# singhhp1069/charon

Hardware: AMD Instinct MI355X
Metric: verified+aggregated 3-of-4 threshold BLS sigs/sec at 1/2/4/8 MI355X (higher is better)
Workload: dtype u32 (Fp 14x28-bit limbs); 1 GPU; config2: 3-of-4, 10000 DVs x 1 attestation per GPU; parallelism=shard1, inflight_launches=3, batches_per_launch=16, rlc_group=16, rlc_chunk=8, gident=0, subgroup_batch=0, level0=passed, hw_queues=4

## Files before the change

charon_amd/csrc/bls_pair.h:

```cpp
#pragma once
#include "bls_lines.h"

namespace tbg {

TBG_HD Fp pair_mul_lane(uint32_t par, const Fp& a, const Fp& ap, const Fp& b, const Fp& bp) {
  const Fp nbp = fp_neg_l(bp);
  return fp_mul2(a, fp_select(par != 0, bp, b), ap, fp_select(par != 0, b, nbp));
}
TBG_HD Fp pair_sqr_lane(uint32_t par, const Fp& a, const Fp& ap) {
  const Fp x = fp_add_l(fp_select(par != 0, ap, a), ap);
  const Fp y = fp_select(par != 0, a, fp_sub_l(a, ap));
  return fp_mul(x, y);
}
TBG_HD Fp pair_conj_lane(uint32_t par, const Fp& a) { return fp_select(par != 0, fp_neg(a), a); }
TBG_HD Fp pair_mul_xi_lane(uint32_t par, const Fp& a, const Fp& ap) {
  return fp_select(par != 0, fp_add(a, ap), fp_sub(a, ap));
}
TBG_HD Fp pair_inv_lane(uint32_t par, const Fp& a, const Fp& ap) {
  const Fp t = fp_inv(fp_mul2(a, a, ap, ap));
  return fp_mul(pair_conj_lane(par, a), t);
}
TBG_HD Fp pair_const(uint32_t par, const Fp2Const& c) { return par ? fp_from_const(c.c1) : fp_from_const(c.c0); }

struct Fp2p { Fp c0, c1; };
// ... 258 lines not shown
TBG_DEV Fp2x px_conj(const Fp2x& a) { return {pair_conj_lane(pair_par(), a.v)}; }
TBG_DEV Fp2x px_mul_xi(const Fp2x& a) { return {pair_mul_xi_lane(pair_par(), a.v, pair_xch(a.v))}; }
TBG_DEV Fp2x px_mul_const(const Fp2x& a, const Fp2Const& c) {
  const uint32_t par = pair_par();
  return {pair_mul_lane(par, a.v, pair_xch(a.v), pair_const(par, c), pair_const(par ^ 1u, c))};
}
TBG_DEV Fp2x rlc_mul_c(const Fp2x& a, const Fp& c) { return {fp_mul(a.v, c)}; }
TBG_DEV Fp2x f_mulfp(const Fp2x& a, const Fp& c) { return {fp_mul(a.v, c)}; }
TBG_DEV Fp2x f_conj(const Fp2x& a) { return px_conj(a); }
TBG_DEV Fp2x f_mulc(const Fp2x& a, const Fp2Const& c) { return px_mul_const(a, c); }
template <> TBG_HD Fp2x f_zero<Fp2x>() { return {fp_zero()}; }
template <> TBG_HD Fp2x f_one<Fp2x>() {
#if defined(__HIP_DEVICE_COMPILE__)
  return {(threadIdx.x & 1u) ? fp_zero() : fp_one()};
#else
  return {fp_one()};
#endif
}

TBG_DEV Fp2x px_load(const Fp2& a) { return {(&a.c0)[pair_par()]}; }
TBG_DEV void px_store(Fp2& dst, const Fp2x& a) { (&dst.c0)[pair_par()] = a.v; }
TBG_DEV Aff<Fp2x> px_load(const G2A& a) { return {px_load(a.x), px_load(a.y)}; }
TBG_DEV Jac<Fp2x> px_load(const G2J& p) { return {px_load(p.X), px_load(p.Y), px_load(p.Z)}; }
TBG_DEV void px_store(G2A& dst, const Aff<Fp2x>& a) { px_store(dst.x, a.x); px_store(dst.y, a.y); }
TBG_DEV void px_store(G2J& dst, const Jac<Fp2x>& p) { px_store(dst.X, p.X); px_store(dst.Y, p.Y); px_store(dst.Z, p.Z); }
TBG_DEV void px_line_store(uint32_t* dst, const LineG<Fp2x>& l) {
  const uint32_t par = pair_par();
  const Fp* f[3] = {&l.l0.v, &l.l1.v, &l.l4.v};
#pragma unroll
  for (int k = 0; k < 3; ++k)
#pragma unroll
    for (int i = 0; i < NL; ++i) dst[(2 * k + par) * NL + i] = f[k]->l[i];
}

template <bool EVAL = true>
TBG_DEV void px_g2_lines(const Aff<Fp2x>& Q, const Fp& nxP, const Fp& yP, uint32_t* out) {
  Jac<Fp2x> T = jac_from_aff(Q);
  const uint32_t par = pair_par();
  uint32_t* dst = out;
  auto sink = [&](int k, const Fp2x& v) {
#pragma unroll
    for (int i = 0; i < NL; ++i) dst[(2 * k + par) * NL + i] = v.v.l[i];
  };
  for (int i = 62; i >= 0; --i) {
    miller_dbl_s<Fp2x, EVAL>(T, nxP, yP, sink);
    dst += LINE_WORDS;
    if ((X_ABS >> i) & 1) {
      miller_add_s<Fp2x, EVAL>(T, Q, nxP, yP, sink);
      dst += LINE_WORDS;
    }
  }
}

TBG_DEV Fp2 px_gather(const Fp2x& a) {
  const Fp o = pair_xch(a.v);
  return pair_par() ? Fp2{o, a.v} : Fp2{a.v, o};
}

}
#endif
```

charon_amd/csrc/bls_row.h:

```cpp
#pragma once
#include "bls_quad.h"

namespace tbg {

#if defined(__HIP_DEVICE_COMPILE__)
constexpr int ROW_N = 1;
#else
constexpr int ROW_N = 16;
#endif

template <class T>
struct RowV {
  T v[ROW_N];
};
using R32 = RowV<int32_t>;
using R64 = RowV<int64_t>;

template <class T, class F>
TBG_HD RowV<T> rmap(F&& f) {
  RowV<T> r;
#pragma unroll
  for (int k = 0; k < ROW_N; ++k) r.v[k] = f(k);
  return r;
}
// ... 451 lines not shown
}
TBG_HD void rl_add5(int r, RowLineSlots& S) {
  if (r >= 4) return;
  R32 a0, a1, b0, b1;
  if (r < 2) { a0 = rl_ld(S, RL_Y); a1 = rl_ld(S, RL_Y + 1); b0 = rl_p(S, 3, 0); b1 = rl_p(S, 3, 1); }
  else {
    a0 = r_norm(rl_p(S, 3, 2) - rl_aX3(S, 0));
    a1 = r_norm(rl_p(S, 3, 3) - rl_aX3(S, 1));
    b0 = rl_R(S, 0);
    b1 = rl_R(S, 1);
  }
  rl_job(S, 4, r, a0, a1, b0, b1);
}
TBG_HD void rl_add6(int r, RowLineSlots& S, int buf) {
  if (r >= 12) return;
  const int c = r & 1, j = r >> 1;
  if (j == 0) row_st(S.s[RL_X + c], row_reduce(rl_aX3(S, c)));
  else if (j == 1) row_st(S.s[RL_Y + c], row_reduce(rl_p(S, 4, 2 + c) - rl_p(S, 4, c)));
  else if (j == 2) row_st(S.s[RL_Z + c], rl_p(S, 2, 2 + c));
  else if (j == 3) row_st(S.l[buf][c], row_reduce(rl_p(S, 3, 6 + c) - rl_p(S, 3, 4 + c)));
  else if (j == 4) row_st(S.l[buf][2 + c], rl_p(S, 2, 6 + c));
  else row_st(S.l[buf][4 + c], rl_p(S, 3, 8 + c));
}

TBG_HD void rl_line_out(const RowLineSlots& S, int buf, int k, uint32_t* dst) {
  const Fp v = fp_from_signed(S.l[buf][k]);
  for (int i = 0; i < NL; ++i) dst[k * NL + i] = v.l[i];
}

template <class Exec, class Out>
TBG_HD void row_g2_lines(Exec& ex, Out& out6, RowLineSlots& S) {
  int idx = 0, buf = 0;
#pragma unroll 1
  for (int i = 62; i >= 0; --i) {
    ex([&](int r) { rl_dbl1(r, S); });
    ex([&](int r) { rl_dbl2(r, S); });
    ex([&](int r) { rl_dbl3(r, S); });
    ex([&](int r) { rl_dbl4(r, S, buf); });
    out6(buf, idx++);
    buf ^= 1;
    if ((X_ABS >> i) & 1) {
      ex([&](int r) { rl_add1(r, S); });
      ex([&](int r) { rl_add2(r, S); });
      ex([&](int r) { rl_add3(r, S); });
      ex([&](int r) { rl_add4(r, S); });
      ex([&](int r) { rl_add5(r, S); });
      ex([&](int r) { rl_add6(r, S, buf); });
      out6(buf, idx++);
      buf ^= 1;
    }
  }
}

}
```

charon_amd/csrc/k_msm.hip:

```cpp
#define TBG_ADD_DBL_INLINE 1
#ifndef TBG_SCHED_FENCE
#define TBG_SCHED_FENCE 1
#endif
#include "tbls_launch.h"
#include "bls_msm.h"
#include "bls_pair.h"
#include "bls_batchinv.h"

namespace tbg {

__global__ void __launch_bounds__(BINV_BLOCK) k_pubkey_tables(const G1A* pk, const G1A* xpk, const int32_t* status,
                                                              uint32_t n, G1A* tab) {
  const uint32_t i = blockIdx.x * blockDim.x + threadIdx.x;
  const bool in = i < n;
  const bool ok = in && status[i] == DEC_OK;
  G1A p0{fp_zero(), fp_zero()}, x0 = p0;
  if (ok) {
    p0 = pk[i];
    x0 = xpk[i];
  }
#if TBG_PK_W2
#pragma unroll 1
  for (int k = 0; k < (int)PK_TAB; ++k) {
    const G1J e = ok ? rlc_key_table_w2_entry(p0, x0, k) : jac_inf<Fp>();
    G1A a{fp_zero(), fp_zero()};
    const bool got = block_jac_to_aff<BINV_WAVES>(e, ok, a);
    if (in) tab[(size_t)PK_TAB * i + k] = got ? a : G1A{fp_zero(), fp_zero()};
  }
#else
  const Fp t = block_batch_inv<BINV_WAVES>(fp_reduce(fp_sub(x0.x, p0.x)), ok);
  if (!in) return;
  G1A ap{fp_zero(), fp_zero()}, am = ap;
  if (ok) rlc_pair_from_inv(p0, x0, t, ap, am);
  tab[2ull * i] = ap;
  tab[2ull * i + 1] = am;
#endif
}

__global__ void TBG_LAUNCH k_rlc_g1_l0(DevBatch B, const G1A* tab, const int32_t* pk_status, uint32_t n_pk) {
  const uint32_t i = blockIdx.x * blockDim.x + threadIdx.x;
  if (i >= B.n_partials || B.partial_status[i] != TBG_PS_NOT_VERIFIED) return;
  const uint32_t pid = B.pubkey_ids[i];
  const bool fused = l0_fused(B);
  if (pid >= n_pk || pk_status[pid] != DEC_OK) {
    B.partial_status[i] = TBG_PS_ERR_PUBKEY;
    if (fused) B.counters[CNT_L0_BAD] = 1;
    return;
  }
  if (fused) {
    const uint4 v = *(const uint4*)(B.l0f_u + 4ull * i);
    const uint32_t uf[4] = {v.x, v.y, v.z, v.w};
    B.part_p[i] = rlc_mul_key_l0f(tab + (size_t)PK_TAB * pid, fp_from_const(G1_BETA), uf);
    return;
  }
  const uint64_t r = rlc_scalar(B.rlc_seed, i);
  uint32_t u[4];
  rlc_digits(r, u);
  B.msm_r[i] = r;
  B.part_p[i] = rlc_mul_key(tab + (size_t)PK_TAB * pid, u);
#pragma unroll
// ... 82 lines not shown
    const int top = 31 - __builtin_clz(m);
#pragma unroll 1
    for (int bit = top - 1; bit >= 0; --bit) {
      acc = jac_dbl_in(acc);
      if ((m >> bit) & 1u) {
        __asm__ __volatile__("" ::: "memory");
        const Jac<Fp2x> b = px_load(B.msm_bkt[j]);
        acc = FAST ? jac_add_x(acc, b, exc) : jac_add(acc, b);
      }
    }
  }
  return acc;
}
#ifndef TBG_MSM_BUCKET_X
#define TBG_MSM_BUCKET_X 1
#endif
__device__ __noinline__ Jac<Fp2x> msm_bucket_complete(const DevBatch& B, uint32_t j) {
  bool unused = false;
  return msm_bucket_scaled<false>(B, j, unused);
}

__global__ void TBG_LAUNCH_N(TBG_PAIR_WAVES) k_msm_bucket(DevBatch B) {
  TBG_URGENT();
  const uint32_t j = (blockIdx.x * blockDim.x + threadIdx.x) >> 1;
  if (j >= MSM_BUCKETS) return;
  if (B.counters[CNT_L0_BAD]) return;
#if TBG_MSM_BUCKET_X
  bool exc = false;
  Jac<Fp2x> acc = msm_bucket_scaled<true>(B, j, exc);
  if (!pair_all(!exc)) acc = msm_bucket_complete(B, j);
#else
  Jac<Fp2x> acc = px_load(B.msm_part[MSM_SPLIT * j]);
#pragma unroll 1
  for (uint32_t sl = 1; sl < MSM_SPLIT; ++sl) acc = jac_add_in<Fp2x, true>(acc, px_load(B.msm_part[MSM_SPLIT * j + sl]));
  const uint32_t m = 2 * j + 1;
  if (m > 1 && !jac_is_inf(acc)) {
    const Jac<Fp2x> b = acc;
    const int top = 31 - __builtin_clz(m);
#pragma unroll 1
    for (int bit = top - 1; bit >= 0; --bit) {
      acc = jac_dbl_in(acc);
      if ((m >> bit) & 1u) acc = jac_add_in<Fp2x, true>(acc, b);
    }
  }
#endif
  px_store(B.msm_bkt[j], acc);
}

constexpr uint32_t MSM_TREE_PAIRS = 128;
constexpr uint32_t MSM_TREE_PER = 4;
constexpr uint32_t MSM_TREE_WG = MSM_BUCKETS / (MSM_TREE_PAIRS * MSM_TREE_PER);
static_assert(MSM_TREE_WG <= 2 * 64 && MSM_TREE_WG <= MSM_SUM_ENTRIES, "second tree kernel: one workgroup");

template <uint32_t PAIRS>
__device__ __forceinline__ Jac<Fp2x> pair_tree_sum(Jac<Fp2x> acc, Jac<Fp2x>* lds) {
  const uint32_t t = threadIdx.x, pr = t >> 1;
#pragma unroll 1
  for (uint32_t s = 1; s < PAIRS; s <<= 1) {
    lds[t] = acc;
    __syncthreads();
    if ((pr & (2 * s - 1)) == 0 && pr + s < PAIRS) acc = jac_add_in<Fp2x, true>(acc, lds[t + 2 * s]);
    __syncthreads();
  }
  return acc;
}

__global__ void __launch_bounds__(2 * MSM_TREE_PAIRS) k_msm_tree(DevBatch B) {
  TBG_URGENT();
  __shared__ Jac<Fp2x> lds[2 * MSM_TREE_PAIRS];
  if (B.counters[CNT_L0_BAD]) return;
  const uint32_t pr = threadIdx.x >> 1;
  const uint32_t a0 = (blockIdx.x * MSM_TREE_PAIRS + pr) * MSM_TREE_PER;
  Jac<Fp2x> acc = px_load(B.msm_bkt[a0]);
#pragma unroll 1
  for (uint32_t a = a0 + 1; a < a0 + MSM_TREE_PER; ++a) acc = jac_add_in<Fp2x, true>(acc, px_load(B.msm_bkt[a]));
  acc = pair_tree_sum<MSM_TREE_PAIRS>(acc, lds);
  if (pr == 0) px_store(B.msm_sum[blockIdx.x], acc);
}

__global__ void __launch_bounds__(MSM_TREE_WG) k_msm_tree_final(DevBatch B) {
  TBG_URGENT();
  constexpr uint32_t PAIRS = MSM_TREE_WG / 2;
  __shared__ Jac<Fp2x> lds[2 * PAIRS];
  if (B.counters[CNT_L0_BAD]) return;
  const uint32_t pr = threadIdx.x >> 1;
  Jac<Fp2x> acc = jac_add_in<Fp2x, true>(px_load(B.msm_sum[2 * pr]), px_load(B.msm_sum[2 * pr + 1]));
  acc = pair_tree_sum<PAIRS>(acc, lds);
  if (pr != 0) return;
  if (jac_is_inf(acc)) {
    if (pair_par() == 0) B.counters[CNT_L0_BAD] = 1;
    return;
  }
  const Fp2x zi = f_inv(acc.Z);
  const Fp2x zi2 = f_sqr(zi);
  px_store(*B.batch_pt, Aff<Fp2x>{f_mul(acc.X, zi2), f_mul(acc.Y, f_mul(zi2, zi))});
}

__global__ void __launch_bounds__(2 * L0F_PAIRS) k_l0f_reduce(DevBatch B, uint32_t n_sg, uint32_t wq, uint32_t n_t) {
  __shared__ Jac<Fp2x> lds[2 * L0F_PAIRS];
  if (B.counters[CNT_L0_BAD]) return;
  const uint32_t pr = threadIdx.x >> 1, b = blockIdx.x;
  const bool qcol = b < SGB_K * wq;
  const uint32_t col = qcol ? b / wq : SGB_K, chunk = qcol ? b % wq : b - SGB_K * wq;
  const uint32_t count = qcol ? n_sg : n_sg * n_t;
  const uint32_t a0 = chunk * L0F_CHUNK + pr * L0F_PER, a1 = min(a0 + L0F_PER, count);
  Jac<Fp2x> acc = jac_inf<Fp2x>();
#pragma unroll 1
  for (uint32_t a = a0; a < a1; ++a) {
    if (qcol) {
      acc = jac_add_in<Fp2x, true>(acc, px_load(B.sgb_part[((size_t)SGB_BUCKETS * a + (size_t)SGB_V * col) * B.sgb_split]));
    } else {
      acc = jac_add_in<Fp2x, true>(acc, px_load(B.sgb_t[a]));
    }
  }
  acc = pair_tree_sum<L0F_PAIRS>(acc, lds);
  if (pr == 0) px_store(B.l0f_sum[b], acc);
}

__global__ void __launch_bounds__(2 * L0F_PAIRS) k_l0f_fold(DevBatch B, uint32_t wq, uint32_t wt) {
  TBG_URGENT();
  __shared__ Jac<Fp2x> lds[2 * L0F_PAIRS];
  if (B.counters[CNT_L0_BAD]) return;
  const uint32_t pr = threadIdx.x >> 1, col = blockIdx.x;
  const uint32_t first = col < SGB_K ? col * wq : SGB_K * wq, count = col < SGB_K ? wq : wt;
  Jac<Fp2x> acc = jac_inf<Fp2x>();
#pragma unroll 1
  for (uint32_t a = pr; a < count; a += L0F_PAIRS) acc = jac_add_in<Fp2x, true>(acc, px_load(B.l0f_sum[first + a]));
  acc = pair_tree_sum<L0F_PAIRS>(acc, lds);
  if (pr == 0) px_store(B.l0f_sum[SGB_K * wq + wt + col], acc);
}

constexpr uint32_t L0F_HORNER_THREADS = 8;
__global__ void __launch_bounds__(64) k_l0f_horner(DevBatch B, uint32_t base) {
  TBG_URGENT();
  __shared__ Jac<Fp2x> lds[L0F_HORNER_THREADS];
  if (B.counters[CNT_L0_BAD]) return;
  const int j = (int)(threadIdx.x >> 1);
  const G2J* tot = B.l0f_sum + base;
  const int e0 = l0f_first(j), e1 = l0f_first(j + 1);
  Jac<Fp2x> acc = px_load(tot[e1 - 1]);
#pragma unroll 1
  for (int e = e1 - 2; e >= e0; --e) acc = l0f_mul13_add(acc, px_load(tot[e]));
  acc = l0f_term(acc, px_load(tot[SGB_K]), j);
  acc = pair_tree_sum<L0F_HORNER_THREADS / 2>(acc, lds);
  if (j != 0) return;
  if (jac_is_inf(acc)) {
    if (pair_par() == 0) B.counters[CNT_L0_BAD] = 1;
    return;
  }
  const Fp2x zi = f_inv(acc.Z);
  const Fp2x zi2 = f_sqr(zi);
  px_store(*B.batch_pt, Aff<Fp2x>{f_mul(acc.X, zi2), f_mul(acc.Y, f_mul(zi2, zi))});
}

void launch_pubkey_tables(const G1A* pk, const G1A* xpk, const int32_t* status, uint32_t n, G1A* tab, hipStream_t st) {
  if (n) TBG_KLAUNCH(k_pubkey_tables, dim3((n + BINV_BLOCK - 1) / BINV_BLOCK), dim3(BINV_BLOCK), st, pk, xpk, status, n,
                     tab);
}

void launch_l0_keys(const DevBatch& B, const G1A* pk_tab, const int32_t* pk_status, uint32_t n_pk, hipStream_t st) {
  if (B.n_partials) TBG_KLAUNCH(k_rlc_g1_l0, grid_for(B.n_partials), dim3(kBlock), st, B, pk_tab, pk_status, n_pk);
}

void launch_l0_msm(const DevBatch& B, hipStream_t st) {
  TBG_KLAUNCH(k_msm_scan, dim3(1), dim3(kScanBlock), st, B);
  if (B.n_partials) TBG_KLAUNCH(k_msm_scatter, grid_for(B.n_partials), dim3(kBlock), st, B);
  TBG_KLAUNCH(k_msm_bucket_part, grid_for(2 * MSM_BUCKETS * MSM_SPLIT), dim3(kBlock), st, B);
  TBG_KLAUNCH(k_msm_bucket, grid_for(2 * MSM_BUCKETS), dim3(kBlock), st, B);
  TBG_KLAUNCH(k_msm_tree, dim3(MSM_TREE_WG), dim3(2 * MSM_TREE_PAIRS), st, B);
  TBG_KLAUNCH(k_msm_tree_final, dim3(1), dim3(MSM_TREE_WG), st, B);
}

void launch_l0_fused_s(const DevBatch& B, hipStream_t st) {
  const uint32_t n_sg = sgb_groups(B.n_partials, B.sgb_m), n_t = sgb_t_slices(B.sgb_m);
  const uint32_t wq = l0f_q_chunks(n_sg), wt = l0f_t_chunks(n_sg, B.sgb_m);
  TBG_KLAUNCH(k_l0f_reduce, dim3(SGB_K * wq + wt), dim3(2 * L0F_PAIRS), st, B, n_sg, wq, n_t);
  TBG_KLAUNCH(k_l0f_fold, dim3(L0F_COLS), dim3(2 * L0F_PAIRS), st, B, wq, wt);
  TBG_KLAUNCH(k_l0f_horner, dim3(1), dim3(L0F_HORNER_THREADS), st, B, SGB_K * wq + wt);
}

}
```

charon_amd/csrc/k_sgb.hip:

```cpp
#define TBG_ADD_DBL_INLINE 1
#ifndef TBG_SCHED_FENCE
#define TBG_SCHED_FENCE 1
#endif
#include "tbls_launch.h"
#include "bls_rlc.h"
#include "bls_pair.h"

namespace tbg {

#ifndef TBG_SGB_SORT_BLOCK
#define TBG_SGB_SORT_BLOCK 256
#endif
constexpr uint32_t kSgbSortBlock = TBG_SGB_SORT_BLOCK;

__global__ void __launch_bounds__(kSgbSortBlock) k_sgb_sort(DevBatch B) {
  __shared__ uint32_t cnt[SGB_BUCKETS];
  __shared__ uint32_t off[SGB_BUCKETS + 1];
  __shared__ int8_t dig[SGB_M * SGB_K];
  const uint32_t g = blockIdx.x, t = threadIdx.x, m = B.sgb_m;
  const uint32_t i0 = g * m;
  const uint32_t n = min(m, B.n_partials - i0);
  for (uint32_t b = t; b < SGB_BUCKETS; b += kSgbSortBlock) cnt[b] = 0;
  if (t == 0) B.sgb_bad[g] = 0;
  const bool fused = l0_fused(B);
// ... 63 lines not shown
  }
  const uint32_t g = w / (SGB_BUCKETS * S), b = (w / S) % SGB_BUCKETS, sl = w % S;
  const uint32_t* goff = B.sgb_off + (size_t)(SGB_BUCKETS + 1) * g;
  const uint32_t o0 = goff[b], n = goff[b + 1] - o0;
  const uint32_t e0 = o0 + (n * sl) / S, e1 = o0 + (n * (sl + 1)) / S;
  const uint32_t* ent = B.sgb_ent + (size_t)m * SGB_K * g;
  const G2A* sig = B.sig_aff + (size_t)m * g;
  Jac<Fp2x> acc = jac_inf<Fp2x>();
#pragma unroll 1
  for (uint32_t e = e0; e < e1; ++e) {
    const uint32_t v = ent[e];
    Aff<Fp2x> p = px_load(sig[v >> 1]);
    p.y = f_reduce(p.y);
    if (v & 1u) p.y = f_reduce(f_neg(p.y));
    acc = jac_add_aff_in(acc, p);
  }
  px_store(B.sgb_part[w], acc);
}

__device__ __forceinline__ void sgb_fail(const DevBatch& B, uint32_t g) {
  B.sgb_bad[g] = 1u;
  if (l0_fused(B)) B.counters[CNT_L0_BAD] = 1u;
}

__global__ void TBG_LAUNCH_N(TBG_PAIR_WAVES) k_sgb_fold(DevBatch B, uint32_t n_sg) {
  const uint32_t w = (blockIdx.x * blockDim.x + threadIdx.x) >> 1;
  if (w >= n_sg * SGB_BUCKETS) return;
  const uint32_t S = B.sgb_split;
  G2J* part = B.sgb_part + (size_t)w * S;
  Jac<Fp2x> acc = px_load(part[0]);
  bool exc = false;
#pragma unroll 1
  for (uint32_t sl = 1; sl < S; ++sl) acc = jac_add_x(acc, px_load(part[sl]), exc);
  if (pair_all(!exc)) px_store(part[0], acc);
  else if (pair_par() == 0) sgb_fail(B, w / SGB_BUCKETS);
}

__global__ void TBG_LAUNCH_N(TBG_PAIR_WAVES) k_sgb_combine(DevBatch B, uint32_t n_sg) {
  const uint32_t w = (blockIdx.x * blockDim.x + threadIdx.x) >> 1;
  if (w >= n_sg * SGB_K) return;
  const uint32_t g = w / SGB_K, k = w % SGB_K, S = B.sgb_split;
  G2J* part = B.sgb_part + ((size_t)SGB_BUCKETS * g + (size_t)SGB_V * k) * S;
  Jac<Fp2x> run = jac_inf<Fp2x>(), q = run;
  bool exc = false;
#pragma unroll 1
  for (int v = (int)SGB_V; v >= 1; --v) {
    run = jac_add_x(run, px_load(part[(size_t)(v - 1) * S]), exc);
    q = jac_add_x(q, run, exc);
  }
  if (pair_all(!exc)) px_store(part[0], q);
  else if (pair_par() == 0) sgb_fail(B, g);
}

__global__ void TBG_LAUNCH_N(TBG_PAIR_WAVES) k_sgb_test(DevBatch B, uint32_t n_sg) {
  const uint32_t w = (blockIdx.x * blockDim.x + threadIdx.x) >> 1;
  if (w >= n_sg * SGB_K) return;
  const uint32_t g = w / SGB_K, k = w % SGB_K;
  const G2J& slot = B.sgb_part[((size_t)SGB_BUCKETS * g + (size_t)SGB_V * k) * B.sgb_split];
  bool ok = true;
  if (!jac_is_inf(px_load(slot))) {
    bool exc = false;
    Jac<Fp2x> m = px_load(slot);
#pragma unroll 1
    for (int i = 62; i >= 0; --i) {
      m = jac_dbl_lo(m);
      if ((X_ABS >> i) & 1) {
        __asm__ __volatile__("" ::: "memory");
        m = jac_add_x(m, px_load(slot), exc);
      }
    }
    if (exc || jac_is_inf(m)) {
      ok = false;
    } else {
      __asm__ __volatile__("" ::: "memory");
      const Jac<Fp2x> ps = g2_psi_g(px_load(slot));
      const Fp2x z1 = f_sqr(ps.Z), z2 = f_sqr(m.Z);
      ok = f_eq(f_mul(ps.X, z2), f_mul(m.X, z1)) &&
           f_eq(f_mul(f_mul(ps.Y, m.Z), z2), f_reduce(f_neg(f_mul(f_mul(m.Y, ps.Z), z1))));
    }
  }
  if (!ok && pair_par() == 0) sgb_fail(B, g);
}

void launch_subgroup_batch(const DevBatch& B, hipStream_t st) {
  if (!B.sgb) return;
  const uint32_t n_sg = sgb_groups(B.n_partials, B.sgb_m);
  if (!n_sg) return;
  TBG_KLAUNCH(k_sgb_sort, dim3(n_sg), dim3(kSgbSortBlock), st, B);
  const uint32_t n_t = l0_fused(B) ? sgb_t_slices(B.sgb_m) : 0u;
  TBG_KLAUNCH(k_sgb_bucket, grid_for(2 * n_sg * (SGB_BUCKETS * B.sgb_split + n_t)), dim3(kBlock), st, B, n_sg, n_t);
  if (B.sgb_split > 1) TBG_KLAUNCH(k_sgb_fold, grid_for(2 * n_sg * SGB_BUCKETS), dim3(kBlock), st, B, n_sg);
  TBG_KLAUNCH(k_sgb_combine, grid_for(2 * n_sg * SGB_K), dim3(kBlock), st, B, n_sg);
  TBG_KLAUNCH(k_sgb_test, grid_for(2 * n_sg * SGB_K), dim3(kBlock), st, B, n_sg);
}

}
```

charon_amd/csrc/tbls_launch.h:

```cpp
#pragma once
#include <hip/hip_runtime.h>
#include "bls_curve.h"
#include "bls_lines.h"
#include "../../include/tbls_gpu.h"

namespace tbg {

constexpr int kBlock = 64;
#ifndef TBG_PK_W2
#define TBG_PK_W2 1
#endif
constexpr uint32_t PK_TAB = TBG_PK_W2 ? 8u : 2u;
#ifndef TBG_REPLAY_SHAPE
#define TBG_REPLAY_SHAPE 1
#endif
#ifndef TBG_L0_SHAPE
#define TBG_L0_SHAPE 1
#endif
#ifndef TBG_L0_SHAPE_WIDE
#define TBG_L0_SHAPE_WIDE 1
#endif
#ifndef TBG_FB_WINDOW
#define TBG_FB_WINDOW 32768u
#endif
// ... 59 lines not shown
  uint32_t* cid_lines;
  uint32_t gident;
  uint32_t* grp_fe;
  uint32_t* gid_list;
  G1A* gid_p;
  uint32_t* gid_lines;
  uint32_t* gid_f;
  uint32_t* id_fe;
  uint32_t* id_list;
  G1A* id_p;
  uint32_t fb_window, fb_base;
  uint32_t fb_full;
  uint32_t* id_lines;
  uint32_t rlc_batch;
  uint64_t* msm_r;
  uint32_t* msm_off;
  uint32_t* msm_cur;
  uint32_t* msm_ent;
  G2J* msm_part;
  G2J* msm_bkt;
  G2J* msm_sum;
  G2A* batch_pt;
  uint32_t* batch_lines;
  uint32_t* batch_f;
  uint32_t* grp_f;
  uint32_t* gm_off;
  uint32_t* gm_ent;
  G2J* gm_part;
  uint32_t* gm_lead;
  uint32_t* gm_list;
  uint32_t* gm_hist;
  uint32_t* gm_order;
  uint32_t sgb;
  uint32_t sgb_m;
  uint32_t sgb_split;
  uint32_t sgb_seed[8];
  uint32_t* sgb_off;
  uint32_t* sgb_ent;
  G2J* sgb_part;
  uint32_t* sgb_bad;
  G2J* sgb_t;
  G2J* l0f_sum;
  uint32_t* l0f_u;
  G2J* agg_acc;
  uint32_t* agg_list;
  int32_t* partial_status;
  int32_t* duty_status;
  uint8_t* agg;
};

enum RlcState : int32_t { RLC_NONE = 0, RLC_COMBINED = 1, RLC_EACH = 2 };
enum GroupState : int32_t { GRP_EMPTY = 0, GRP_LINES = 1, GRP_OK = 2, GRP_FAIL = 3, GRP_GID = 4 };
enum Counter : int { CNT_DUTIES = 0, CNT_PARTIALS = 1, CNT_AGG = 2, CNT_CHUNKS = 3, CNT_CID = 4, CNT_L0_BAD = 5,
                     CNT_L0_OK = 6, CNT_GID = 7, CNT_LAZY = 8, CNT_WORDS = 9 };

constexpr uint32_t MSM_BUCKETS = 32768;
constexpr uint32_t MSM_SPLIT = 4;
constexpr uint32_t MSM_SUM_ENTRIES = 128;
#ifndef TBG_SGB_M
#define TBG_SGB_M 1024
#endif
#ifndef TBG_SGB_SPLIT
#define TBG_SGB_SPLIT 4
#endif
constexpr uint32_t SGB_M = TBG_SGB_M;
constexpr uint32_t SGB_M_MIN = 64;
constexpr uint32_t SGB_K = 18;
constexpr uint32_t SGB_V = 6;
constexpr uint32_t SGB_BUCKETS = SGB_K * SGB_V;
constexpr uint32_t SGB_SPLIT = TBG_SGB_SPLIT;
constexpr uint32_t SGB_MIN_PARTIALS = 2 * SGB_M;
TBG_HD uint32_t sgb_groups(uint32_t n_partials, uint32_t m) { return (n_partials + m - 1) / m; }
TBG_HD uint32_t sgb_split_for(uint32_t m) {
  const uint32_t s = SGB_SPLIT * m / SGB_M;
  return s ? s : 1u;
}
TBG_HD bool l0_fused(const DevBatch& B) {
  return TBG_PK_W2 && B.rlc_batch && B.rlc_group && B.sgb && B.n_partials;
}
constexpr uint32_t SGB_T_PER = 32;
TBG_HD uint32_t sgb_t_slices(uint32_t m) { return m / SGB_T_PER; }
constexpr uint32_t L0F_COLS = SGB_K + 1;
constexpr uint32_t L0F_PAIRS = 128, L0F_PER = 4;
constexpr uint32_t L0F_CHUNK = L0F_PAIRS * L0F_PER;
TBG_HD uint32_t l0f_q_chunks(uint32_t n_sg) { return (n_sg + L0F_CHUNK - 1) / L0F_CHUNK; }
TBG_HD uint32_t l0f_t_chunks(uint32_t n_sg, uint32_t m) { return (n_sg * sgb_t_slices(m) + L0F_CHUNK - 1) / L0F_CHUNK; }
TBG_HD uint32_t l0f_sum_entries(uint32_t n_sg, uint32_t m) {
  return SGB_K * l0f_q_chunks(n_sg) + l0f_t_chunks(n_sg, m) + L0F_COLS;
}
constexpr uint32_t L0_TREE_FAN = 4;
TBG_HD uint32_t grp_f_entries(uint32_t n_groups) { return n_groups + n_groups / (L0_TREE_FAN - 1) + 40; }
enum MillerMode : int { MILLER_GROUPS = 0, MILLER_L0 = 1, MILLER_GROUP_S = 2 };
enum DutySumPhase : int { DSUM_BOTH = 0, DSUM_L0_P = 1, DSUM_FALLBACK_S = 2, DSUM_P = 3 };
#ifndef TBG_GMSM
#define TBG_GMSM 1
#endif
constexpr uint32_t GM_W = 4, GM_V = 8, GM_BUCKETS = GM_W * GM_V;

constexpr uint32_t CHUNK_DEGENERATE = 0x80000000u;
constexpr uint32_t ID_DEGENERATE = 0x80000000u;
enum FoldKind : int { FOLD_GROUPS = 0, FOLD_CHUNKS = 1, FOLD_CID = 2, FOLD_IDENT = 3, FOLD_GID = 5 };

TBG_HD bool fb_in_pass(const DevBatch& B, uint32_t k) { return B.fb_window == 0 || k - B.fb_base < B.fb_window; }
TBG_HD size_t fb_slot(const DevBatch& B, uint32_t k) { return (size_t)LINES_WORDS * (k - B.fb_base); }
template <class F>
TBG_HD void fb_pass_loop(const DevBatch& B, uint32_t first, uint32_t stride, uint32_t count, F&& body) {
  const uint32_t w = B.fb_window ? B.fb_window : 0xFFFFFFFFu;
// ... 82 lines not shown
```

Baseline: 3.402 million DV-duties/s (n verifies + 1 aggregate each).

## Fuse subgroup test into l0f reduce and row-parallelize Horner combine

Folds the per-subgroup psi test into the l0f reduce launch as extra workgroups, so one kernel launch and its serialization point go away. It also replaces the 8-thread pairwise Horner kernel with a row-parallel version that runs four chains at once over 640 threads with shared-memory slots. The old kernel stays as a fallback, gated on a new counter that is set when the sum hits infinity. This adds a launch and more LDS use, and the row-form formulas carry correctness risk.

```diff
diff --git a/charon_amd/csrc/bls_pair.h b/charon_amd/csrc/bls_pair.h
--- a/charon_amd/csrc/bls_pair.h
+++ b/charon_amd/csrc/bls_pair.h
@@ -334,6 +334,19 @@
   }
 }
 
+template <uint32_t PAIRS>
+TBG_DEV Jac<Fp2x> pair_tree_sum(Jac<Fp2x> acc, Jac<Fp2x>* lds) {
+  const uint32_t t = threadIdx.x, pr = t >> 1;
+#pragma unroll 1
+  for (uint32_t s = 1; s < PAIRS; s <<= 1) {
+    lds[t] = acc;
+    __syncthreads();
+    if ((pr & (2 * s - 1)) == 0 && pr + s < PAIRS) acc = jac_add_in<Fp2x, true>(acc, lds[t + 2 * s]);
+    __syncthreads();
+  }
+  return acc;
+}
+
 TBG_DEV Fp2 px_gather(const Fp2x& a) {
   const Fp o = pair_xch(a.v);
   return pair_par() ? Fp2{o, a.v} : Fp2{a.v, o};
diff --git a/charon_amd/csrc/bls_row.h b/charon_amd/csrc/bls_row.h
--- a/charon_amd/csrc/bls_row.h
+++ b/charon_amd/csrc/bls_row.h
@@ -527,4 +527,190 @@
   }
 }
 
-}
+constexpr int RG_ROWS = 10;
+struct RowG2Slots {
+  int32_t pt[4][6][16];
+  int32_t p[5][10][16];
+};
+enum { RG_X = 0, RG_Y = 2, RG_Z = 4 };
+TBG_HD R32 rg_ld(const RowG2Slots& S, int pt, int i) { return row_ld(S.pt[pt][i]); }
+TBG_HD R32 rg_p(const RowG2Slots& S, int ph, int i) { return row_ld(S.p[ph][i]); }
+TBG_HD void rg_job(RowG2Slots& S, int ph, int r, const R32& a0, const R32& a1, const R32& b0, const R32& b1) {
+#if defined(TBG_BOUNDS_CHECK) && !defined(__HIP_DEVICE_COMPILE__)
+  for (int k = 0; k < ROW_N; ++k) {
+    const int64_t lim = (int64_t)1 << 29;
+    TBG_BOUND(a0.v[k] <= lim && a0.v[k] >= -lim && a1.v[k] <= lim && a1.v[k] >= -lim, "rg_job a limbs <= 2^29");
+    TBG_BOUND(b0.v[k] <= lim && b0.v[k] >= -lim && b1.v[k] <= lim && b1.v[k] >= -lim, "rg_job b limbs <= 2^29");
+  }
+#endif
+  row_st(S.p[ph][r], row_fp2_mul_c(r & 1, a0, a1, b0, b1));
+}
+
+TBG_HD void rg_add1(int r, RowG2Slots& S, int a, int b) {
+  if (r >= 10) return;
+  const int j = r >> 1;
+  const int pa = (j == 1 || j == 4) ? b : a, ia = j < 3 ? RG_Z : RG_Y;
+  const int pb = (j == 0 || j == 4) ? a : b;
+  rg_job(S, 0, r, rg_ld(S, pa, ia), rg_ld(S, pa, ia + 1), rg_ld(S, pb, RG_Z), rg_ld(S, pb, RG_Z + 1));
+}
+TBG_HD void rg_add2(int r, RowG2Slots& S, int a, int b) {
+  if (r >= 8) return;
+  const int j = r >> 1;
+  R32 a0, a1;
+  if (j == 0) { a0 = rg_ld(S, a, RG_X); a1 = rg_ld(S, a, RG_X + 1); }
+  else if (j == 1) { a0 = rg_ld(S, b, RG_X); a1 = rg_ld(S, b, RG_X + 1); }
+  else if (j == 2) { a0 = rg_p(S, 0, 6); a1 = rg_p(S, 0, 7); }
+  else { a0 = rg_p(S, 0, 8); a1 = rg_p(S, 0, 9); }
+  const int zz = (j & 1) ? 0 : 2;
+  rg_job(S, 1, r, a0, a1, rg_p(S, 0, zz), rg_p(S, 0, zz + 1));
+}
+TBG_HD R32 rg_H(const RowG2Slots& S, int c) { return r_norm(rg_p(S, 1, 2 + c) - rg_p(S, 1, c)); }
+TBG_HD R32 rg_R(const RowG2Slots& S, int c) { return r_norm(rg_p(S, 1, 6 + c) - rg_p(S, 1, 4 + c)); }
+TBG_HD void rg_add3(int r, RowG2Slots& S) {
+  if (r >= 6) return;
+  const int j = r >> 1;
+  R32 a0, a1, b0, b1;
+  if (j == 0) { a0 = b0 = rg_H(S, 0); a1 = b1 = rg_H(S, 1); }
+  else if (j == 1) { a0 = rg_p(S, 0, 4); a1 = rg_p(S, 0, 5); b0 = rg_H(S, 0); b1 = rg_H(S, 1); }
+  else { a0 = b0 = rg_R(S, 0); a1 = b1 = rg_R(S, 1); }
+  rg_job(S, 2, r, a0, a1, b0, b1);
+}
+TBG_HD void rg_add4(int r, RowG2Slots& S) {
+  if (r >= 4) return;
+  R32 a0, a1;
+  if (r < 2) { a0 = rg_H(S, 0); a1 = rg_H(S, 1); }
+  else { a0 = rg_p(S, 1, 0); a1 = rg_p(S, 1, 1); }
+  rg_job(S, 3, r, a0, a1, rg_p(S, 2, 0), rg_p(S, 2, 1));
+}
+TBG_HD R32 rg_aX3(const RowG2Slots& S, int c) {
+  return r_norm(rg_p(S, 2, 4 + c) - rg_p(S, 3, c) - r_mul_small(rg_p(S, 3, 2 + c), 2));
+}
+TBG_HD void rg_add5(int r, RowG2Slots& S) {
+  if (r >= 4) return;
+  R32 a0, a1, b0, b1;
+  if (r < 2) { a0 = rg_p(S, 1, 4); a1 = rg_p(S, 1, 5); b0 = rg_p(S, 3, 0); b1 = rg_p(S, 3, 1); }
+  else {
+    a0 = r_norm(rg_p(S, 3, 2) - rg_aX3(S, 0));
+    a1 = r_norm(rg_p(S, 3, 3) - rg_aX3(S, 1));
+    b0 = rg_R(S, 0);
+    b1 = rg_R(S, 1);
+  }
+  rg_job(S, 4, r, a0, a1, b0, b1);
+}
+TBG_HD void rg_add6(int r, RowG2Slots& S, int d) {
+  if (r >= 6) return;
+  const int c = r & 1, j = r >> 1;
+  if (j == 0) row_st(S.pt[d][RG_X + c], row_reduce(rg_aX3(S, c)));
+  else if (j == 1) row_st(S.pt[d][RG_Y + c], row_reduce(rg_p(S, 4, 2 + c) - rg_p(S, 4, c)));
+  else row_st(S.pt[d][RG_Z + c], rg_p(S, 2, 2 + c));
+}
+
+TBG_HD void rg_dbl1(int r, RowG2Slots& S, int a) {
+  if (r >= 6) return;
+  const int j = r >> 1;
+  const int ia = j == 0 ? RG_X : RG_Y, ib = j == 0 ? RG_X : (j == 1 ? RG_Y : RG_Z);
+  rg_job(S, 0, r, rg_ld(S, a, ia), rg_ld(S, a, ia + 1), rg_ld(S, a, ib), rg_ld(S, a, ib + 1));
+}
+TBG_HD void rg_dbl2(int r, RowG2Slots& S, int a) {
+  if (r >= 6) return;
+  const int j = r >> 1;
+  R32 a0, a1;
+  if (j == 0) { a0 = rg_p(S, 0, 2); a1 = rg_p(S, 0, 3); }
+  else if (j == 1) { a0 = rg_ld(S, a, RG_X) + rg_p(S, 0, 2); a1 = rg_ld(S, a, RG_X + 1) + rg_p(S, 0, 3); }
+  else { a0 = r_norm(r_mul_small(rg_p(S, 0, 0), 3)); a1 = r_norm(r_mul_small(rg_p(S, 0, 1), 3)); }
+  rg_job(S, 1, r, a0, a1, a0, a1);
+}
+TBG_HD R32 rg_D(const RowG2Slots& S, int c) {
+  return r_norm(r_mul_small(rg_p(S, 1, 2 + c) - rg_p(S, 0, c) - rg_p(S, 1, c), 2));
+}
+TBG_HD R32 rg_dX3(const RowG2Slots& S, int c) { return r_norm(rg_p(S, 1, 4 + c) - r_mul_small(rg_D(S, c), 2)); }
+TBG_HD void rg_dbl3(int r, RowG2Slots& S) {
+  if (r >= 2) return;
+  rg_job(S, 2, r, r_norm(rg_D(S, 0) - rg_dX3(S, 0)), r_norm(rg_D(S, 1) - rg_dX3(S, 1)),
+         r_norm(r_mul_small(rg_p(S, 0, 0), 3)), r_norm(r_mul_small(rg_p(S, 0, 1), 3)));
+}
+TBG_HD void rg_dbl4(int r, RowG2Slots& S, int d) {
+  if (r >= 6) return;
+  const int c = r & 1, j = r >> 1;
+  if (j == 0) row_st(S.pt[d][RG_X + c], row_reduce(rg_dX3(S, c)));
+  else if (j == 1) row_st(S.pt[d][RG_Y + c], row_reduce(rg_p(S, 2, c) - r_mul_small(r_norm(r_mul_small(rg_p(S, 1, c), 4)), 2)));
+  else row_st(S.pt[d][RG_Z + c], row_reduce(r_mul_small(rg_p(S, 0, 4 + c), 2)));
+}
+
+TBG_HD void rg_psi(int r, RowG2Slots& S, int d, int a) {
+  if (r >= 6) return;
+  const int c = r & 1, j = r >> 1;
+  if (j == 2) {
+    const R32 z = rg_ld(S, a, RG_Z + c);
+    row_st(S.pt[d][RG_Z + c], rsel(c == 0, z, -z));
+    return;
+  }
+  const R32 k0 = j == 0 ? r_limbs(PSI_X.c0) : r_limbs(PSI_Y.c0), k1 = j == 0 ? r_limbs(PSI_X.c1) : r_limbs(PSI_Y.c1);
+  row_st(S.pt[d][2 * j + c], row_fp2_mul_c(c, rg_ld(S, a, 2 * j), -rg_ld(S, a, 2 * j + 1), k0, k1));
+}
+TBG_HD void rg_load(int r, RowG2Slots& S, int d, const uint32_t* src) {
+  if (r < 6) row_st(S.pt[d][r], row_from_limbs(src + r * NL));
+}
+TBG_HD void rg_copy(int r, RowG2Slots& S, int d, const RowG2Slots& Sa, int a) {
+  if (r < 6) row_st(S.pt[d][r], row_ld(Sa.pt[a][r]));
+}
+
+template <class Exec>
+TBG_HD void rg_add(Exec& ex, RowG2Slots* S, uint32_t m, int d, int a, int b) {
+  auto on = [&](int r) { return ((m >> (r / RG_ROWS)) & 1u) != 0; };
+  ex([&](int r) { if (on(r)) rg_add1(r % RG_ROWS, S[r / RG_ROWS], a, b); });
+  ex([&](int r) { if (on(r)) rg_add2(r % RG_ROWS, S[r / RG_ROWS], a, b); });
+  ex([&](int r) { if (on(r)) rg_add3(r % RG_ROWS, S[r / RG_ROWS]); });
+  ex([&](int r) { if (on(r)) rg_add4(r % RG_ROWS, S[r / RG_ROWS]); });
+  ex([&](int r) { if (on(r)) rg_add5(r % RG_ROWS, S[r / RG_ROWS]); });
+  ex([&](int r) { if (on(r)) rg_add6(r % RG_ROWS, S[r / RG_ROWS], d); });
+}
+template <class Exec>
+TBG_HD void rg_dbl(Exec& ex, RowG2Slots* S, uint32_t m, int d, int a) {
+  auto on = [&](int r) { return ((m >> (r / RG_ROWS)) & 1u) != 0; };
+  ex([&](int r) { if (on(r)) rg_dbl1(r % RG_ROWS, S[r / RG_ROWS], a); });
+  ex([&](int r) { if (on(r)) rg_dbl2(r % RG_ROWS, S[r / RG_ROWS], a); });
+  ex([&](int r) { if (on(r)) rg_dbl3(r % RG_ROWS, S[r / RG_ROWS]); });
+  ex([&](int r) { if (on(r)) rg_dbl4(r % RG_ROWS, S[r / RG_ROWS], d); });
+}
+
+enum { RG_ACC = 0, RG_T = 1, RG_Q = 2, RG_TT = 3 };
+constexpr int L0F_ROW_CHAINS = 4;
+TBG_HD constexpr int l0f_row_first(int j) { return j < 2 ? 5 * j : 10 + 4 * (j - 2); }
+template <class Exec>
+TBG_HD void row_l0f_s(Exec& ex, RowG2Slots* S, const uint32_t* tot) {
+  constexpr int PW = 6 * NL;
+  ex([&](int r) {
+    const int g = r / RG_ROWS, lr = r % RG_ROWS;
+    rg_load(lr, S[g], RG_ACC, tot + (size_t)PW * (l0f_row_first(g + 1) - 1));
+  });
+  ex([&](int r) { rg_load(r % RG_ROWS, S[r / RG_ROWS], RG_TT, tot + (size_t)PW * 18); });
+#pragma unroll 1
+  for (int s = 0; s < 4; ++s) {
+    const uint32_t m = s == 0 ? 3u : 15u;
+    ex([&](int r) {
+      const int g = r / RG_ROWS, lr = r % RG_ROWS;
+      const int e = l0f_row_first(g + 1) - 2 - (s - (g >= 2 ? 1 : 0));
+      if ((m >> g) & 1u) rg_load(lr, S[g], RG_Q, tot + (size_t)PW * e);
+    });
+    rg_dbl(ex, S, m, RG_T, RG_ACC);
+    rg_add(ex, S, m, RG_T, RG_T, RG_ACC);
+    rg_dbl(ex, S, m, RG_T, RG_T);
+    rg_dbl(ex, S, m, RG_T, RG_T);
+    rg_add(ex, S, m, RG_T, RG_T, RG_ACC);
+    rg_add(ex, S, m, RG_ACC, RG_T, RG_Q);
+  }
+  rg_dbl(ex, S, 15u, RG_T, RG_ACC);
+  rg_add(ex, S, 15u, RG_ACC, RG_T, RG_TT);
+#pragma unroll 1
+  for (int k = 0; k < 3; ++k) {
+    ex([&](int r) { if (r / RG_ROWS > k) rg_psi(r % RG_ROWS, S[r / RG_ROWS], RG_T, RG_ACC); });
+    ex([&](int r) { if (r / RG_ROWS > k) rg_copy(r % RG_ROWS, S[r / RG_ROWS], RG_ACC, S[r / RG_ROWS], RG_T); });
+  }
+  ex([&](int r) { const int g = r / RG_ROWS; if (g == 0 || g == 2) rg_copy(r % RG_ROWS, S[g], RG_Q, S[g + 1], RG_ACC); });
+  rg_add(ex, S, 5u, RG_ACC, RG_ACC, RG_Q);
+  ex([&](int r) { if (r / RG_ROWS == 0) rg_copy(r % RG_ROWS, S[0], RG_Q, S[2], RG_ACC); });
+  rg_add(ex, S, 1u, RG_ACC, RG_ACC, RG_Q);
+}
+
+}
diff --git a/charon_amd/csrc/k_msm.hip b/charon_amd/csrc/k_msm.hip
--- a/charon_amd/csrc/k_msm.hip
+++ b/charon_amd/csrc/k_msm.hip
@@ -6,6 +6,7 @@
 #include "bls_msm.h"
 #include "bls_pair.h"
 #include "bls_batchinv.h"
+#include "bls_row.h"
 
 namespace tbg {
 
@@ -194,19 +195,6 @@
 constexpr uint32_t MSM_TREE_WG = MSM_BUCKETS / (MSM_TREE_PAIRS * MSM_TREE_PER);
 static_assert(MSM_TREE_WG <= 2 * 64 && MSM_TREE_WG <= MSM_SUM_ENTRIES, "second tree kernel: one workgroup");
 
-template <uint32_t PAIRS>
-__device__ __forceinline__ Jac<Fp2x> pair_tree_sum(Jac<Fp2x> acc, Jac<Fp2x>* lds) {
-  const uint32_t t = threadIdx.x, pr = t >> 1;
-#pragma unroll 1
-  for (uint32_t s = 1; s < PAIRS; s <<= 1) {
-    lds[t] = acc;
-    __syncthreads();
-    if ((pr & (2 * s - 1)) == 0 && pr + s < PAIRS) acc = jac_add_in<Fp2x, true>(acc, lds[t + 2 * s]);
-    __syncthreads();
-  }
-  return acc;
-}
-
 __global__ void __launch_bounds__(2 * MSM_TREE_PAIRS) k_msm_tree(DevBatch B) {
   TBG_URGENT();
   __shared__ Jac<Fp2x> lds[2 * MSM_TREE_PAIRS];
@@ -238,27 +226,6 @@
   px_store(*B.batch_pt, Aff<Fp2x>{f_mul(acc.X, zi2), f_mul(acc.Y, f_mul(zi2, zi))});
 }
 
-__global__ void __launch_bounds__(2 * L0F_PAIRS) k_l0f_reduce(DevBatch B, uint32_t n_sg, uint32_t wq, uint32_t n_t) {
-  __shared__ Jac<Fp2x> lds[2 * L0F_PAIRS];
-  if (B.counters[CNT_L0_BAD]) return;
-  const uint32_t pr = threadIdx.x >> 1, b = blockIdx.x;
-  const bool qcol = b < SGB_K * wq;
-  const uint32_t col = qcol ? b / wq : SGB_K, chunk = qcol ? b % wq : b - SGB_K * wq;
-  const uint32_t count = qcol ? n_sg : n_sg * n_t;
-  const uint32_t a0 = chunk * L0F_CHUNK + pr * L0F_PER, a1 = min(a0 + L0F_PER, count);
-  Jac<Fp2x> acc = jac_inf<Fp2x>();
-#pragma unroll 1
-  for (uint32_t a = a0; a < a1; ++a) {
-    if (qcol) {
-      acc = jac_add_in<Fp2x, true>(acc, px_load(B.sgb_part[((size_t)SGB_BUCKETS * a + (size_t)SGB_V * col) * B.sgb_split]));
-    } else {
-      acc = jac_add_in<Fp2x, true>(acc, px_load(B.sgb_t[a]));
-    }
-  }
-  acc = pair_tree_sum<L0F_PAIRS>(acc, lds);
-  if (pr == 0) px_store(B.l0f_sum[b], acc);
-}
-
 __global__ void __launch_bounds__(2 * L0F_PAIRS) k_l0f_fold(DevBatch B, uint32_t wq, uint32_t wt) {
   TBG_URGENT();
   __shared__ Jac<Fp2x> lds[2 * L0F_PAIRS];
@@ -272,11 +239,35 @@
   if (pr == 0) px_store(B.l0f_sum[SGB_K * wq + wt + col], acc);
 }
 
+static_assert(L0F_ROW_CHAINS == 4 && SGB_K == 18, "row_l0f_s: four dimensions, 18 columns and T");
+static_assert(l0f_row_first(1) == 5 && l0f_row_first(2) == 10 && l0f_row_first(3) == 14 && l0f_row_first(4) == 18,
+              "row_l0f_s's columns per dimension");
+constexpr uint32_t L0F_ROW_THREADS = L0F_ROW_CHAINS * RG_ROWS * 16;
+__global__ void __launch_bounds__(L0F_ROW_THREADS) k_l0f_horner(DevBatch B, uint32_t base) {
+  TBG_URGENT();
+  __shared__ RowG2Slots S[L0F_ROW_CHAINS];
+  __shared__ G2J sum;
+  if (B.counters[CNT_L0_BAD]) return;
+  RowDevExec ex;
+  row_l0f_s(ex, S, (const uint32_t*)(B.l0f_sum + base));
+  if (threadIdx.x < 6) ((Fp*)&sum)[threadIdx.x] = fp_from_signed(S[0].pt[RG_ACC][threadIdx.x]);
+  __syncthreads();
+  if (threadIdx.x >= 2) return;
+  const Jac<Fp2x> acc = px_load(sum);
+  if (jac_is_inf(acc)) {
+    if (pair_par() == 0) B.counters[CNT_L0F_PAIR] = 1;
+    return;
+  }
+  const Fp2x zi = f_inv(acc.Z);
+  const Fp2x zi2 = f_sqr(zi);
+  px_store(*B.batch_pt, Aff<Fp2x>{f_mul(acc.X, zi2), f_mul(acc.Y, f_mul(zi2, zi))});
+}
+
 constexpr uint32_t L0F_HORNER_THREADS = 8;
-__global__ void __launch_bounds__(64) k_l0f_horner(DevBatch B, uint32_t base) {
+__global__ void __launch_bounds__(64) k_l0f_horner_x(DevBatch B, uint32_t base) {
   TBG_URGENT();
   __shared__ Jac<Fp2x> lds[L0F_HORNER_THREADS];
-  if (B.counters[CNT_L0_BAD]) return;
+  if (B.counters[CNT_L0_BAD] || !B.counters[CNT_L0F_PAIR]) return;
   const int j = (int)(threadIdx.x >> 1);
   const G2J* tot = B.l0f_sum + base;
   const int e0 = l0f_first(j), e1 = l0f_first(j + 1);
@@ -314,11 +305,11 @@
 }
 
 void launch_l0_fused_s(const DevBatch& B, hipStream_t st) {
-  const uint32_t n_sg = sgb_groups(B.n_partials, B.sgb_m), n_t = sgb_t_slices(B.sgb_m);
+  const uint32_t n_sg = sgb_groups(B.n_partials, B.sgb_m);
   const uint32_t wq = l0f_q_chunks(n_sg), wt = l0f_t_chunks(n_sg, B.sgb_m);
-  TBG_KLAUNCH(k_l0f_reduce, dim3(SGB_K * wq + wt), dim3(2 * L0F_PAIRS), st, B, n_sg, wq, n_t);
   TBG_KLAUNCH(k_l0f_fold, dim3(L0F_COLS), dim3(2 * L0F_PAIRS), st, B, wq, wt);
-  TBG_KLAUNCH(k_l0f_horner, dim3(1), dim3(L0F_HORNER_THREADS), st, B, SGB_K * wq + wt);
-}
-
-}
+  TBG_KLAUNCH(k_l0f_horner, dim3(1), dim3(L0F_ROW_THREADS), st, B, SGB_K * wq + wt);
+  TBG_KLAUNCH(k_l0f_horner_x, dim3(1), dim3(L0F_HORNER_THREADS), st, B, SGB_K * wq + wt);
+}
+
+}
diff --git a/charon_amd/csrc/k_sgb.hip b/charon_amd/csrc/k_sgb.hip
--- a/charon_amd/csrc/k_sgb.hip
+++ b/charon_amd/csrc/k_sgb.hip
@@ -139,8 +139,7 @@
   else if (pair_par() == 0) sgb_fail(B, g);
 }
 
-__global__ void TBG_LAUNCH_N(TBG_PAIR_WAVES) k_sgb_test(DevBatch B, uint32_t n_sg) {
-  const uint32_t w = (blockIdx.x * blockDim.x + threadIdx.x) >> 1;
+__device__ __forceinline__ void sgb_test_pair(const DevBatch& B, uint32_t n_sg, uint32_t w) {
   if (w >= n_sg * SGB_K) return;
   const uint32_t g = w / SGB_K, k = w % SGB_K;
   const G2J& slot = B.sgb_part[((size_t)SGB_BUCKETS * g + (size_t)SGB_V * k) * B.sgb_split];
@@ -167,6 +166,36 @@
     }
   }
   if (!ok && pair_par() == 0) sgb_fail(B, g);
+}
+
+__global__ void TBG_LAUNCH_N(TBG_PAIR_WAVES) k_sgb_test(DevBatch B, uint32_t n_sg) {
+  sgb_test_pair(B, n_sg, (blockIdx.x * blockDim.x + threadIdx.x) >> 1);
+}
+
+__global__ void __launch_bounds__(2 * L0F_PAIRS, TBG_PAIR_WAVES)
+    k_l0f_reduce(DevBatch B, uint32_t n_sg, uint32_t n_test_wg, uint32_t wq, uint32_t n_t) {
+  __shared__ Jac<Fp2x> lds[2 * L0F_PAIRS];
+  const uint32_t pr = threadIdx.x >> 1;
+  if (blockIdx.x < n_test_wg) {
+    sgb_test_pair(B, n_sg, blockIdx.x * L0F_PAIRS + pr);
+    return;
+  }
+  const uint32_t b = blockIdx.x - n_test_wg;
+  const bool qcol = b < SGB_K * wq;
+  const uint32_t col = qcol ? b / wq : SGB_K, chunk = qcol ? b % wq : b - SGB_K * wq;
+  const uint32_t count = qcol ? n_sg : n_sg * n_t;
+  const uint32_t a0 = chunk * L0F_CHUNK + pr * L0F_PER, a1 = min(a0 + L0F_PER, count);
+  Jac<Fp2x> acc = jac_inf<Fp2x>();
+#pragma unroll 1
+  for (uint32_t a = a0; a < a1; ++a) {
+    if (qcol) {
+      acc = jac_add_in<Fp2x, true>(acc, px_load(B.sgb_part[((size_t)SGB_BUCKETS * a + (size_t)SGB_V * col) * B.sgb_split]));
+    } else {
+      acc = jac_add_in<Fp2x, true>(acc, px_load(B.sgb_t[a]));
+    }
+  }
+  acc = pair_tree_sum<L0F_PAIRS>(acc, lds);
+  if (pr == 0) px_store(B.l0f_sum[b], acc);
 }
 
 void launch_subgroup_batch(const DevBatch& B, hipStream_t st) {
@@ -178,7 +207,13 @@
   TBG_KLAUNCH(k_sgb_bucket, grid_for(2 * n_sg * (SGB_BUCKETS * B.sgb_split + n_t)), dim3(kBlock), st, B, n_sg, n_t);
   if (B.sgb_split > 1) TBG_KLAUNCH(k_sgb_fold, grid_for(2 * n_sg * SGB_BUCKETS), dim3(kBlock), st, B, n_sg);
   TBG_KLAUNCH(k_sgb_combine, grid_for(2 * n_sg * SGB_K), dim3(kBlock), st, B, n_sg);
-  TBG_KLAUNCH(k_sgb_test, grid_for(2 * n_sg * SGB_K), dim3(kBlock), st, B, n_sg);
-}
-
-}
+  if (!l0_fused(B)) {
+    TBG_KLAUNCH(k_sgb_test, grid_for(2 * n_sg * SGB_K), dim3(kBlock), st, B, n_sg);
+    return;
+  }
+  const uint32_t n_test_wg = (n_sg * SGB_K + L0F_PAIRS - 1) / L0F_PAIRS;
+  const uint32_t wq = l0f_q_chunks(n_sg), wt = l0f_t_chunks(n_sg, B.sgb_m);
+  TBG_KLAUNCH(k_l0f_reduce, dim3(n_test_wg + SGB_K * wq + wt), dim3(2 * L0F_PAIRS), st, B, n_sg, n_test_wg, wq, n_t);
+}
+
+}
diff --git a/charon_amd/csrc/tbls_launch.h b/charon_amd/csrc/tbls_launch.h
--- a/charon_amd/csrc/tbls_launch.h
+++ b/charon_amd/csrc/tbls_launch.h
@@ -135,7 +135,7 @@
 enum RlcState : int32_t { RLC_NONE = 0, RLC_COMBINED = 1, RLC_EACH = 2 };
 enum GroupState : int32_t { GRP_EMPTY = 0, GRP_LINES = 1, GRP_OK = 2, GRP_FAIL = 3, GRP_GID = 4 };
 enum Counter : int { CNT_DUTIES = 0, CNT_PARTIALS = 1, CNT_AGG = 2, CNT_CHUNKS = 3, CNT_CID = 4, CNT_L0_BAD = 5,
-                     CNT_L0_OK = 6, CNT_GID = 7, CNT_LAZY = 8, CNT_WORDS = 9 };
+                     CNT_L0_OK = 6, CNT_GID = 7, CNT_LAZY = 8, CNT_L0F_PAIR = 9, CNT_WORDS = 10 };
 
 constexpr uint32_t MSM_BUCKETS = 32768;
 constexpr uint32_t MSM_SPLIT = 4;
```

Result: no change. 3.426 million DV-duties/s (n verifies + 1 aggregate each), median of 6 (+0.7%).
